# pasqal-io/Pulser

Measured on AMD Instinct MI355X. Metric: sim-us/sec, 14-atom Rydberg anneal sequence, sesolve fp64 (aggregate over independent sequences), higher is better.
Workload: dtype f64; 1 GPU; north star: 14-atom triangular register (2 x 7 at R_b), analog Ising anneal 3100 ns, sesolve complex128; step = the full 3.1 us for a batch of different sequences per GPU; n_atoms=14, sequences_per_gpu=256, parallelism=dp1

## Files before the change

pulser_amd/csrc/k_split_reg.hpp:

```cpp

#ifndef SPLITR_TRIG
#define SPLITR_TRIG 256
#endif
#ifndef SPLITR_KO
#define SPLITR_KO 0
#endif
#ifndef SPLITR_TMODE
#define SPLITR_TMODE 1
#endif
#ifndef SPLITR_GMODE
#define SPLITR_GMODE 0
#endif
#ifndef SPLITR_WMODE
#define SPLITR_WMODE 1
#endif
#ifndef SPLITR_EMODE
#define SPLITR_EMODE 0
#endif
#ifndef SPLITR_KWARM
#define SPLITR_KWARM 1
#endif
#ifndef SPLITR_PREF
#define SPLITR_PREF 0
#endif
#ifndef SPLITR_LATE
#define SPLITR_LATE 1
#endif
#ifndef SPLITR_P5
#define SPLITR_P5 0
#endif
#ifndef SPLITR_LATE_REAL
#define SPLITR_LATE_REAL 0
#endif
#ifndef SPLITR_YCHAIN
#define SPLITR_YCHAIN 1
#endif
#include "split_ychain.hpp"

template <int N, int NR>
struct SplitRegLayout {
  static constexpr int NW = N - 6 - NR;
  static constexpr int NTB = NR - NW;
  static constexpr int ND = 6 - NTB;
  static_assert(NW >= 0 && NW <= 3 && NTB >= 2 && ND >= 1 && ND <= 4, "unsupported shape");
  static constexpr bool kXchg = SPLITR_TMODE != 3;
  __host__ __device__ static constexpr int regbit(bool odd, int j) {
    if (!odd) return 6 + NW + j;
    return j < NW ? 6 + j : (kXchg ? ND + (j - NW) : 6 + NW + j);
  }
  __host__ __device__ static constexpr int lanebit(bool odd, int j) {
    if (j < ND || !odd || !kXchg) return j;
    return 6 + 2 * NW + (j - ND);
  }
  __host__ __device__ static constexpr int wavebit(bool odd, int j) { return odd ? 6 + NW + j : 6 + j; }
  __host__ __device__ static constexpr unsigned index(bool odd, unsigned t, unsigned r) {
    unsigned i = 0;
    for (int j = 0; j < 6; ++j) i |= ((t >> j) & 1u) << lanebit(odd, j);
    for (int j = 0; j < NW; ++j) i |= ((t >> (6 + j)) & 1u) << wavebit(odd, j);
    for (int j = 0; j < NR; ++j) i |= ((r >> j) & 1u) << regbit(odd, j);
    return i;
  }
  static constexpr int FM = ND == 4 ? 0 : (ND == 3 ? 2 : 3);
  __host__ __device__ static constexpr int swz(int y) { return ND == 3 ? ((y >> 1) & 1) : (y & FM); }
};

template <int I, int E, class Fn>
__device__ __forceinline__ void splitr_for(Fn&& f) {
  if constexpr (I < E) {
    f(std::integral_constant<int, I>{});
    splitr_for<I + 1, E>(f);
  }
}
template <int V>
using splitr_c = std::integral_constant<int, V>;
__host__ __device__ constexpr int splitr_low_clear(int v) {
  int j = 0;
  while (v & (1 << j)) ++j;
  return j;
}

template <int CTRL>
__device__ __forceinline__ double splitr_dpp(double v) {
  const int lo = __builtin_amdgcn_update_dpp(0, __double2loint(v), CTRL, 0xF, 0xF, true);
  const int hi = __builtin_amdgcn_update_dpp(0, __double2hiint(v), CTRL, 0xF, 0xF, true);
  return __hiloint2double(hi, lo);
}
#ifndef SPLITR_B2
#define SPLITR_B2 0
#endif
#ifndef SPLITR_HM
#define SPLITR_HM 1
#endif
template <int ND>
__device__ __forceinline__ unsigned splitr_lane(unsigned t) { return (SPLITR_HM && ND >= 3) ? t ^ ((t & 4u) ? 3u : 0u) : t; }
template <int F>
__device__ __forceinline__ double splitr_partner(double v) {
  if constexpr (F == 0) return splitr_dpp<0xB1>(v);
  else if constexpr (F == 1) return splitr_dpp<0x4E>(v);
  else if constexpr (F == 3) return splitr_dpp<0x128>(v);
  else if constexpr (SPLITR_HM == 1) return splitr_dpp<0x141>(v);
  else if constexpr (SPLITR_B2 == 1) {
    const int lo = __builtin_amdgcn_ds_swizzle(__double2loint(v), 0x101F);
    const int hi = __builtin_amdgcn_ds_swizzle(__double2hiint(v), 0x101F);
    return __hiloint2double(hi, lo);
  }
  else return splitr_dpp<0x1B>(splitr_dpp<0x141>(v));
}

template <int N, int NR, bool DECAY, bool ROWS = false, bool CPLX = false, bool SNAP = false>
__global__ __launch_bounds__(64 << (N - 6 - NR)) __attribute__((amdgpu_waves_per_eu(1, NR >= 6 ? 1 : 2))) void k_split_reg(const SplitArgs A, const SplitRun R, long long stage_stride) {
  static_assert(!(SNAP && (ROWS || DECAY)), "snapshots inside a run: plain ket runs only");
  typedef SplitRegLayout<N, NR> L;
  constexpr int NW = L::NW, NTB = L::NTB, ND = L::ND;
  constexpr int NT = 64 << NW;
  constexpr int NA = 1 << NR;
  constexpr int PW = (1 << NW) - 1;
  constexpr int CH = NA / 4;
  constexpr int NG = 1 << NW;
  constexpr int GR = 1 << NTB;
  constexpr int NBUF = CH / GR;
  extern __shared__ __attribute__((aligned(16))) char smem[];
  cplx* pbuf = reinterpret_cast<cplx*>(smem);
  cplx* trig = pbuf + 2 * NT * CH;
  cplx* gtab = trig + SPLITR_TRIG;
  double* wtab = reinterpret_cast<double*>(gtab + (NT / 64) * NA);
  double* etab = wtab + (SPLIT_MAX_SUB * SPLIT_MAX_STAGES + 2);

  const unsigned t = threadIdx.x;
  const unsigned l = t & 63u, w = t >> 6;
  const unsigned tq = splitr_lane<ND>(t);
  const int b = ROWS ? (int)blockIdx.z : (int)blockIdx.y;
  const int n_pre = R.kick_pre != 0.0 ? 1 : 0;
  const int n_stages = splitrun_first(R, R.nsub) + 1 + n_pre;
  const double csgn = (ROWS && A.conj) ? -1.0 : 1.0;
  const double* __restrict__ coefs = A.ccur + (size_t)b * N * 4;
  const double* __restrict__ e0 = A.e0 + (size_t)b * A.e0_stride;

  if (SPLITR_WMODE) {
    for (int jj = (int)t; jj < n_stages; jj += NT) {
      const int j = jj - n_pre;
      wtab[jj] = j < 0 ? 0.0 : splitrun_weight(R, j);
    }
  }
  for (unsigned k = t; k < SPLITR_TRIG; k += NT) {
    double sn, cs;
    sincospi((double)k * (2.0 / SPLITR_TRIG), &sn, &cs);
    trig[k] = make_double2(cs, sn);
  }
  double et[2], ev[2][NR], eg[2];
#pragma unroll
  for (int o = 0; o < 2; ++o) {
    et[o] = e0[L::index(o, tq, NA - 1)];
#pragma unroll
    for (int j = 0; j < NR; ++j) ev[o][j] = e0[L::index(o, tq, (NA - 1) ^ (1u << j))] - et[o];
    eg[o] = e0[L::index(o, NT - 1, l & (NA - 1))];
    if (SPLITR_EMODE) {
      etab[(2 * o) * NT + t] = et[o];
      etab[(2 * o + 1) * NT + t] = eg[o];
    }
  }
  double* ftl = etab + (SPLITR_EMODE ? 4 * NT : 0);
  unsigned a_row = 0;
  auto row_factor = [&](int which, unsigned col_bits, unsigned mask) -> double {
    const unsigned a = a_row;
    const int n11 = __popc(a & col_bits & mask), n10 = __popc(a & ~col_bits & mask), n01 = __popc(~a & col_bits & mask);
    const int n00 = __popc(mask) - n11 - n10 - n01;
    const double* tb = ftl + 64 * which;
    return tb[n00] * tb[16 + n01] * tb[32 + n10] * tb[48 + n11];
  };
  if (ROWS && (A.use_pre || A.use_post) && t < 128) ftl[t] = A.ftab[t];
  __syncthreads();
  typedef const __attribute__((address_space(4))) double* cptr_t;
  auto expmi = [&](double phi) -> cplx {
    const double kk = rint(phi * (SPLITR_TRIG / 6.283185307179586));
    double rr = fma(-kk, 6.283185307179586 / SPLITR_TRIG, phi);
    rr = fma(-kk, 2.4492935982947064e-16 / SPLITR_TRIG, rr);
    const cplx tb = trig[((int)kk) & (SPLITR_TRIG - 1)];
    const double r2 = rr * rr;
    double cr, sr;
    if (SPLITR_TRIG >= 512) {
      cr = fma(r2, fma(r2, 4.1666666666666664e-02, -0.5), 1.0);
      sr = rr * fma(r2, fma(r2, 8.333333333333333e-03, -1.6666666666666666e-01), 1.0);
    } else {
      cr = fma(r2, fma(r2, fma(r2, -1.3888888888888889e-03, 4.1666666666666664e-02), -0.5), 1.0);
      sr = rr * fma(r2, fma(r2, fma(r2, -1.984126984126984e-04, 8.333333333333333e-03), -1.6666666666666666e-01), 1.0);
    }
    return make_double2(fma(tb.x, cr, -tb.y * sr), -fma(tb.y, cr, tb.x * sr));
  };
  auto cm = [](cplx a, cplx c) -> cplx { return make_double2(fma(a.x, c.x, -a.y * c.y), fma(a.x, c.y, a.y * c.x)); };
  cplx* __restrict__ const tslice = pbuf + 64 * w;
  const unsigned la = l & ((1u << ND) - 1u), lT = l >> ND;

  for (unsigned row = ROWS ? blockIdx.y : 0u; row < (ROWS ? (1u << N) : 1u); row += ROWS ? gridDim.y : 1u) {
  a_row = row;
  cplx* __restrict__ st = A.state + ((((size_t)b << (ROWS ? N : 0)) + (ROWS ? row : 0u)) << N);
  if (ROWS) __syncthreads();
  if (ROWS && A.use_pre && t < NA) ftl[128 + t] = row_factor(0, L::index(false, 0u, t), L::index(false, 0u, NA - 1));
  if (ROWS && A.use_pre) __syncthreads();
  double xr[NA], xi[NA];
  {
    const double fl = (ROWS && A.use_pre) ? row_factor(0, L::index(false, tq, 0u), L::index(false, NT - 1, 0u)) : 1.0;
    splitr_for<0, NA>([&](auto Rc) {
      constexpr int r = decltype(Rc)::value;
      const cplx v = st[L::index(false, tq, r)];
      const double f = (ROWS && A.use_pre) ? fl * ftl[128 + r] : 1.0;
      xr[r] = v.x * f;
      xi[r] = v.y * (ROWS ? f * csgn : f);
    });
  }


  auto rot_reg = [&](auto J, double T, double U, auto MASK, auto VAL) {
    if (SPLITR_KO & 16) return;
    splitr_for<0, NA>([&](auto Rc) {
      constexpr int r = decltype(Rc)::value, j = decltype(J)::value;
      if constexpr ((r & decltype(MASK)::value) == decltype(VAL)::value && !(r & (1 << j))) {
        constexpr int q = r | (1 << j);
        const double a0x = xr[r], a0y = xi[r], a1x = xr[q], a1y = xi[q];
        if constexpr (CPLX) {
          xr[r] = fma(-U, a1x, fma(-T, a1y, a0x));
          xi[r] = fma(-U, a1y, fma(T, a1x, a0y));
          xr[q] = fma(U, a0x, fma(-T, a0y, a1x));
          xi[q] = fma(U, a0y, fma(T, a0x, a1y));
        } else {
          xr[r] = fma(-T, a1y, a0x);
          xi[r] = fma(T, a1x, a0y);
          xr[q] = fma(-T, a0y, a1x);
          xi[q] = fma(T, a0x, a1y);
        }
      }
    });
  };

  double cprod = 1.0;
  bool odd = false;
  double Dn[6 + NW + NR], wEn = 0.0;
  auto load_next = [&](int sn, bool oddn) {
    cptr_t cn = (cptr_t)(unsigned long long)(coefs + (size_t)sn * stage_stride);
#pragma unroll
    for (int j = 0; j < 6; ++j) Dn[j] = cn[4 * (N - 1 - (oddn ? L::lanebit(true, j) : L::lanebit(false, j))) + 3];
#pragma unroll
    for (int j = 0; j < NW; ++j) Dn[6 + j] = cn[4 * (N - 1 - (oddn ? L::wavebit(true, j) : L::wavebit(false, j))) + 3];
#pragma unroll
    for (int j = 0; j < NR; ++j) Dn[6 + NW + j] = cn[4 * (N - 1 - (oddn ? L::regbit(true, j) : L::regbit(false, j))) + 3];
    if (SPLITR_WMODE) wEn = uniform_d(wtab[sn]);
  };
  if (SPLITR_PREF) load_next(0, false);
  unsigned warm = 0;
  auto stage = [&](const int sg, auto plain_close_t) {
    constexpr bool PLAIN_CLOSE = decltype(plain_close_t)::value;
    cptr_t c4 = (cptr_t)(unsigned long long)(coefs + (size_t)sg * stage_stride);
    auto coef = [&](int bit_even, int bit_odd, int field) -> double {
      const int p = odd ? bit_odd : bit_even;
      return c4[4 * (N - 1 - p) + field];
    };
    double Tl[6], Dl[6], Tw[NW > 0 ? NW : 1], Dw[NW > 0 ? NW : 1], Tr[NR], Dr[NR];
    double Ul[6], Uw[NW > 0 ? NW : 1], Ur[NR];
    constexpr int TF = CPLX ? 2 : 1;
    double cnext = 1.0;
#pragma unroll
    for (int j = 0; j < 6; ++j) Dl[j] = SPLITR_PREF ? Dn[j] : coef(L::lanebit(false, j), L::lanebit(true, j), 3);
#pragma unroll
    for (int j = 0; j < NW; ++j) Dw[j] = SPLITR_PREF ? Dn[6 + j] : coef(L::wavebit(false, j), L::wavebit(true, j), 3);
#pragma unroll
    for (int j = 0; j < NR; ++j) Dr[j] = SPLITR_PREF ? Dn[6 + NW + j] : coef(L::regbit(false, j), L::regbit(true, j), 3);
    auto load_rot = [&](cptr_t cl) {
      auto coefl = [&](int bit_even, int bit_odd, int field) -> double {
        const int p = odd ? bit_odd : bit_even;
        return cl[4 * (N - 1 - p) + field];
      };
#pragma unroll
      for (int j = 0; j < 6; ++j) {
        Tl[j] = coefl(L::lanebit(false, j), L::lanebit(true, j), TF);
        Ul[j] = CPLX ? coefl(L::lanebit(false, j), L::lanebit(true, j), 1) : 0.0;
        cnext *= coefl(L::lanebit(false, j), L::lanebit(true, j), 0);
      }
#pragma unroll
      for (int j = 0; j < NW; ++j) {
        Tw[j] = coefl(L::wavebit(false, j), L::wavebit(true, j), TF);
        Uw[j] = CPLX ? coefl(L::wavebit(false, j), L::wavebit(true, j), 1) : 0.0;
        cnext *= coefl(L::wavebit(false, j), L::wavebit(true, j), 0);
      }
#pragma unroll
      for (int j = 0; j < NR; ++j) {
        Tr[j] = coefl(L::regbit(false, j), L::regbit(true, j), TF);
        Ur[j] = CPLX ? coefl(L::regbit(false, j), L::regbit(true, j), 1) : 0.0;
        cnext *= coefl(L::regbit(false, j), L::regbit(true, j), 0);
      }
    };
    constexpr bool kLate = (SPLITR_LATE && CPLX) || (SPLITR_LATE_REAL && !CPLX);
    if (!kLate && !PLAIN_CLOSE) load_rot(c4);
    double wE;
    if (SPLITR_WMODE && SPLITR_PREF) {
      wE = wEn;
    } else if (SPLITR_WMODE) {
      wE = uniform_d(wtab[sg]);
    } else {
      const int sj = sg - n_pre;
      wE = sj < 0 ? 0.0 : splitrun_weight(R, sj);
    }
    double et_s, eg_s;
    if (SPLITR_EMODE) {
      et_s = etab[(odd ? 2 : 0) * NT + t];
      eg_s = etab[(odd ? 3 : 1) * NT + t];
    } else {
      et_s = odd ? et[1] : et[0];
      eg_s = odd ? eg[1] : eg[0];
    }

    cplx Bf, F[NR], Gl;
    if (!(SPLITR_KO & 8)) {
      double dthr = 0.0;
#pragma unroll
      for (int j = 0; j < 6; ++j) dthr += ((tq >> j) & 1u) ? 0.0 : Dl[j];
#pragma unroll
      for (int j = 0; j < NW; ++j) dthr += ((tq >> (6 + j)) & 1u) ? 0.0 : Dw[j];
      Bf = expmi(fma(wE, et_s, -dthr));
      double sc = cprod;
      if (DECAY)
        sc *= exp(wE * (A.dec_a + A.dec_b * (double)(__popc(tq) + NR)));
      Bf = make_double2(Bf.x * sc, Bf.y * sc);
      const double dF = DECAY ? exp(-wE * A.dec_b) : 1.0;
#pragma unroll
      for (int j = 0; j < NR; ++j) {
        F[j] = expmi(fma(wE, odd ? ev[1][j] : ev[0][j], -Dr[j]));
        if (DECAY) F[j] = make_double2(F[j].x * dF, F[j].y * dF);
      }
      Gl = expmi(wE * eg_s);
      if (!SPLITR_GMODE) {
        gtab[w * NA + (l & (NA - 1))] = Gl;
        __builtin_amdgcn_wave_barrier();
      }
    }
    if (kLate && !PLAIN_CLOSE) {
      unsigned long long cl = (unsigned long long)(coefs + (size_t)sg * stage_stride);
      asm volatile("" : "+s"(cl));
      load_rot((cptr_t)cl);
    }
    cprod = cnext;
    const cplx* __restrict__ gw = gtab + w * NA;
    auto gval = [&](auto Rc) -> cplx {
      constexpr int r = decltype(Rc)::value;
      if (SPLITR_GMODE) {
        const int a = __builtin_amdgcn_readlane(__double2loint(Gl.x), r), b2 = __builtin_amdgcn_readlane(__double2hiint(Gl.x), r);
        const int c = __builtin_amdgcn_readlane(__double2loint(Gl.y), r), d = __builtin_amdgcn_readlane(__double2hiint(Gl.y), r);
        return make_double2(__hiloint2double(b2, a), __hiloint2double(d, c));
      }
      return gw[r];
    };

    cplx Pg[NG];
    auto phase_group = [&](auto Gc) {
      constexpr int g = decltype(Gc)::value;
      if (SPLITR_KO & 8) return;
      if constexpr (g == NG - 1) Pg[g] = Bf;
      else Pg[g] = cm(Pg[g | (1 << splitr_low_clear(g))], F[splitr_low_clear(g)]);
      cplx Pt[GR];
      splitr_for<0, GR>([&](auto Ic) {
        constexpr int rho = GR - 1 - decltype(Ic)::value;
        if constexpr (rho == GR - 1) Pt[rho] = Pg[g];
        else Pt[rho] = cm(Pt[rho | (1 << splitr_low_clear(rho))], F[NW + splitr_low_clear(rho)]);
        constexpr int r = g | (rho << NW);
        const cplx q = cm(Pt[rho], gval(splitr_c<r>{}));
        const double ax = xr[r], ay = xi[r];
        xr[r] = fma(ax, q.x, -ay * q.y);
        xi[r] = fma(ax, q.y, ay * q.x);
      });
    };
    constexpr bool kP5 = SPLITR_P5 && SPLITR_TMODE == 1 && NTB == 2 && NW > 0 && !(SPLITR_KO & 4);
    auto swap_d = [](double& a, double& c, auto is32) {
      unsigned alo = (unsigned)__double2loint(a), ahi = (unsigned)__double2hiint(a);
      unsigned clo = (unsigned)__double2loint(c), chi = (unsigned)__double2hiint(c);
      if constexpr (decltype(is32)::value) {
        auto p = __builtin_amdgcn_permlane32_swap(alo, clo, false, false);
        auto q = __builtin_amdgcn_permlane32_swap(ahi, chi, false, false);
        alo = p[0]; clo = p[1]; ahi = q[0]; chi = q[1];
      } else {
        auto p = __builtin_amdgcn_permlane16_swap(alo, clo, false, false);
        auto q = __builtin_amdgcn_permlane16_swap(ahi, chi, false, false);
        alo = p[0]; clo = p[1]; ahi = q[0]; chi = q[1];
      }
      a = __hiloint2double((int)ahi, (int)alo);
      c = __hiloint2double((int)chi, (int)clo);
    };
    constexpr bool kYChain = SPLITR_YCHAIN != 0 && !CPLX && SPLITR_HM == 1 && SPLITR_TMODE == 1 && !SPLITR_B2 && !(SPLITR_KO & 2) && ND >= 2;
    constexpr bool kYStore = kYChain && SPLITR_YCHAIN == 2 && NW > 0 && !kP5 && !(SPLITR_KO & 4);
    auto t_swap = [&](auto Gc) {
      constexpr int g = decltype(Gc)::value;
      if (SPLITR_KO & 1) return;
      constexpr int r0 = g, r1 = g | (1 << NW), r2 = g | (2 << NW), r3 = g | (3 << NW);
      swap_d(xr[r0], xr[r1], std::false_type{}); swap_d(xi[r0], xi[r1], std::false_type{});
      swap_d(xr[r2], xr[r3], std::false_type{}); swap_d(xi[r2], xi[r3], std::false_type{});
      if constexpr (!kP5) {
        swap_d(xr[r0], xr[r2], std::true_type{}); swap_d(xi[r0], xi[r2], std::true_type{});
        swap_d(xr[r1], xr[r3], std::true_type{}); swap_d(xi[r1], xi[r3], std::true_type{});
      }
    };
    auto t_write = [&](auto Gc) {
      constexpr int g = decltype(Gc)::value;
      if (SPLITR_KO & 1) return;
      splitr_for<0, GR>([&](auto Ic) {
        constexpr int rho = decltype(Ic)::value;
        constexpr int run = rho + (NBUF == 2 ? (g & 1) * GR : 0);
        tslice[64 * NG * run + la + ((lT ^ (unsigned)L::swz(rho)) << ND)] = make_double2(xr[g | (rho << NW)], xi[g | (rho << NW)]);
      });
    };
    auto t_read = [&](auto Gc) {
      constexpr int g = decltype(Gc)::value;
      if (SPLITR_KO & 1) return;
      __builtin_amdgcn_wave_barrier();
      const unsigned run = lT + (NBUF == 2 ? (g & 1) * GR : 0);
      splitr_for<0, GR>([&](auto Ic) {
        constexpr int rho = decltype(Ic)::value;
        const cplx v = tslice[64 * NG * run + la + (((unsigned)rho ^ (unsigned)L::swz((int)lT)) << ND)];
        xr[g | (rho << NW)] = v.x;
        xi[g | (rho << NW)] = v.y;
      });
    };
    auto rot_t_old = [&](auto Gc) {
      splitr_for<0, NTB>([&](auto Mc) {
        constexpr int m = decltype(Mc)::value;
        rot_reg(splitr_c<NW + m>{}, Tr[NW + m], Ur[NW + m], splitr_c<PW>{}, Gc);
      });
    };
    auto rot_t_new = [&](auto Gc) {
      splitr_for<0, (kP5 ? 1 : NTB)>([&](auto Mc) {
        constexpr int m = decltype(Mc)::value;
        rot_reg(splitr_c<NW + m>{}, Tl[ND + m], Ul[ND + m], splitr_c<PW>{}, Gc);
      });
    };
    double Us[6] = {0.0, 0.0, 0.0, 0.0, 0.0, 0.0};
    if constexpr (CPLX) {
#pragma unroll
      for (int j = 0; j < 6; ++j) Us[j] = ((tq >> j) & 1u) ? Ul[j] : -Ul[j];
    }
    auto xpartner = [&](double v, auto Jc) -> double {
      int lo = __double2loint(v), hi = __double2hiint(v);
      if constexpr (decltype(Jc)::value == 4) {
        lo = __builtin_amdgcn_ds_swizzle(lo, 0x401F);
        hi = __builtin_amdgcn_ds_swizzle(hi, 0x401F);
      } else {
        const int addr = (int)((l ^ 32u) << 2);
        lo = __builtin_amdgcn_ds_bpermute(addr, lo);
        hi = __builtin_amdgcn_ds_bpermute(addr, hi);
      }
      return __hiloint2double(hi, lo);
    };
    auto rot_lane_x = [&](auto Rc) {
      constexpr int r = decltype(Rc)::value;
      if (SPLITR_KO & 1) return;
      splitr_for<4, 6>([&](auto Jc) {
        constexpr int j = decltype(Jc)::value;
        const double T = Tl[j], px = xpartner(xr[r], Jc), py = xpartner(xi[r], Jc);
        if constexpr (CPLX) {
          xr[r] = fma(Us[j], px, fma(-T, py, xr[r]));
          xi[r] = fma(Us[j], py, fma(T, px, xi[r]));
        } else {
          xr[r] = fma(-T, py, xr[r]);
          xi[r] = fma(T, px, xi[r]);
        }
      });
    };
    auto rot_lane = [&](auto Rc, auto MASK) {
      constexpr int r = decltype(Rc)::value, mask = decltype(MASK)::value;
      if (SPLITR_KO & 2) return;
      if constexpr (ND > 0 && (mask & 1)) {
        const double T = Tl[0], px = splitr_partner<0>(xr[r]), py = splitr_partner<0>(xi[r]);
        if constexpr (CPLX) {
          xr[r] = fma(Us[0], px, fma(-T, py, xr[r]));
          xi[r] = fma(Us[0], py, fma(T, px, xi[r]));
        } else {
          xr[r] = fma(-T, py, xr[r]);
          xi[r] = fma(T, px, xi[r]);
        }
      }
      if constexpr (ND > 1 && (mask & 2)) {
        const double T = Tl[1], px = splitr_partner<1>(xr[r]), py = splitr_partner<1>(xi[r]);
        if constexpr (CPLX) {
          xr[r] = fma(Us[1], px, fma(-T, py, xr[r]));
          xi[r] = fma(Us[1], py, fma(T, px, xi[r]));
        } else {
          xr[r] = fma(-T, py, xr[r]);
          xi[r] = fma(T, px, xi[r]);
        }
      }
      if constexpr (ND > 3 && (mask & 8)) {
        const double T = Tl[3], px = splitr_partner<3>(xr[r]), py = splitr_partner<3>(xi[r]);
        if constexpr (CPLX) {
          xr[r] = fma(Us[3], px, fma(-T, py, xr[r]));
          xi[r] = fma(Us[3], py, fma(T, px, xi[r]));
        } else {
          xr[r] = fma(-T, py, xr[r]);
          xi[r] = fma(T, px, xi[r]);
        }
      }
      if constexpr (ND > 2 && (mask & 4)) {
        const double T = Tl[2], px = splitr_partner<2>(xr[r]), py = splitr_partner<2>(xi[r]);
        if constexpr (CPLX) {
          xr[r] = fma(Us[2], px, fma(-T, py, xr[r]));
          xi[r] = fma(Us[2], py, fma(T, px, xi[r]));
        } else {
          xr[r] = fma(-T, py, xr[r]);
          xi[r] = fma(T, px, xi[r]);
        }
      }
    };
    if constexpr (PLAIN_CLOSE) {
      splitr_for<0, NG>([&](auto Ic) { phase_group(splitr_c<(NG - 1 - decltype(Ic)::value)>{}); });
    } else {
    constexpr int TMASK = SPLITR_TMODE == 2 ? 3 : 0;
    constexpr int PMASK = ((1 << ND) - 1) & ~TMASK;
    if constexpr (SPLITR_TMODE == 2) {
      splitr_for<0, NG>([&](auto Ic) { phase_group(splitr_c<(NG - 1 - decltype(Ic)::value)>{}); });
      splitr_for<0, NG>([&](auto Ic) {
        constexpr int g = NG - 1 - decltype(Ic)::value;
        rot_t_old(splitr_c<g>{});
        splitr_for<0, GR>([&](auto Qc) { rot_lane(splitr_c<(g | (decltype(Qc)::value << NW))>{}, splitr_c<TMASK>{}); });
        t_write(splitr_c<g>{});
        t_read(splitr_c<g>{});
        if constexpr (g + 1 < NG) rot_t_new(splitr_c<g + 1>{});
      });
      rot_t_new(splitr_c<0>{});
    } else {
      splitr_for<0, NG>([&](auto Ic) {
        constexpr int g = NG - 1 - decltype(Ic)::value;
        phase_group(splitr_c<g>{});
        rot_t_old(splitr_c<g>{});
        if constexpr (SPLITR_TMODE == 3) {
        } else if constexpr (SPLITR_TMODE == 1 && NTB == 2) {
          t_swap(splitr_c<g>{});
          rot_t_new(splitr_c<g>{});
        } else {
          t_write(splitr_c<g>{});
          t_read(splitr_c<g>{});
          if constexpr (g + 1 < NG) rot_t_new(splitr_c<g + 1>{});
        }
      });
      if constexpr (!(SPLITR_TMODE == 1 && NTB == 2) && SPLITR_TMODE != 3) rot_t_new(splitr_c<0>{});
    }

    constexpr int CM = 3 << (NR - 2);
    auto pre_regs = [&](auto Cc) {
      constexpr int c = decltype(Cc)::value;
      splitr_for<0, NW>([&](auto Jc) { rot_reg(Jc, Tr[decltype(Jc)::value], Ur[decltype(Jc)::value], splitr_c<CM>{}, splitr_c<(c << (NR - 2))>{}); });
    };
    auto chain_step = [&](auto Cc, auto Ic) {
      constexpr int c = decltype(Cc)::value, i = decltype(Ic)::value;
      typedef SplitYPlan<ND, (kYStore ? 1 : 0)> PL;
      constexpr SplitYHop h = PL::hops[i];
      if constexpr (h.n > 0) splitr_for<0, CH>([&](auto Kc) { constexpr int r = decltype(Kc)::value | (c << (NR - 2)); xi[r] = splitr_dpp<h.ctrl[0]>(xi[r]); });
      if constexpr (h.n > 1) splitr_for<0, CH>([&](auto Kc) { constexpr int r = decltype(Kc)::value | (c << (NR - 2)); xi[r] = splitr_dpp<h.ctrl[1]>(xi[r]); });
      if constexpr (i < ND) {
        const double T = Tl[PL::order[i < ND ? i : 0]];
        splitr_for<0, CH>([&](auto Kc) {
          constexpr int r = decltype(Kc)::value | (c << (NR - 2));
          const double x0 = xr[r];
          xr[r] = fma(-T, xi[r], x0);
          xi[r] = fma(T, x0, xi[r]);
        });
      }
    };
    auto pre = [&](auto Cc) {
      constexpr int c = decltype(Cc)::value;
      pre_regs(Cc);
      if constexpr (kYChain) {
        splitr_for<0, ND + 1>([&](auto Ic) { chain_step(Cc, Ic); });
      } else {
        splitr_for<0, CH>([&](auto Kc) {
          rot_lane(splitr_c<(decltype(Kc)::value | (c << (NR - 2)))>{}, splitr_c<PMASK>{});
          if constexpr (SPLITR_TMODE == 3) rot_lane_x(splitr_c<(decltype(Kc)::value | (c << (NR - 2)))>{});
        });
      }
    };
    auto post = [&](auto Cc) {
      constexpr int c = decltype(Cc)::value;
      splitr_for<0, NW>([&](auto Jc) { rot_reg(Jc, Tw[decltype(Jc)::value], Uw[decltype(Jc)::value], splitr_c<CM>{}, splitr_c<(c << (NR - 2))>{}); });
    };
    auto pass_write_part = [&](auto Cc, auto K0c, auto K1c) {
      constexpr int c = decltype(Cc)::value, K0 = decltype(K0c)::value, K1 = decltype(K1c)::value;
      if constexpr (kYStore) {
        constexpr unsigned S = SplitYPlan<ND, 1>::final_shift;
        double* __restrict__ px = reinterpret_cast<double*>(pbuf + (c & 1) * (NT * CH) + t);
        double* __restrict__ py = reinterpret_cast<double*>(pbuf + (c & 1) * (NT * CH) + (t ^ S)) + 1;
        splitr_for<K0, K1>([&](auto Kc) {
          constexpr int k = decltype(Kc)::value, kp = k & PW, ks = k >> NW;
          px[2 * 64 * NG * (kp + NG * ks)] = xr[k | (c << (NR - 2))];
          py[2 * 64 * NG * (kp + NG * ks)] = xi[k | (c << (NR - 2))];
        });
        return;
      }
      cplx* __restrict__ pb = pbuf + (c & 1) * (NT * CH) + t;
      splitr_for<K0, K1>([&](auto Kc) {
        constexpr int k = decltype(Kc)::value, kp = k & PW, ks = k >> NW;
        pb[64 * NG * (kp + NG * ks)] = make_double2(xr[k | (c << (NR - 2))], xi[k | (c << (NR - 2))]);
      });
    };
    auto pass_write = [&](auto Cc) { pass_write_part(Cc, splitr_c<0>{}, splitr_c<CH>{}); };
    auto write_pre = [&](auto Cw, auto Cp) {
      if constexpr (kYChain) {
        pre_regs(Cp);
        splitr_for<0, ND + 1>([&](auto Ic) {
          constexpr int i = decltype(Ic)::value;
          pass_write_part(Cw, splitr_c<(i * CH / (ND + 1))>{}, splitr_c<((i + 1) * CH / (ND + 1))>{});
          __builtin_amdgcn_sched_barrier(0);
          chain_step(Cp, Ic);
          __builtin_amdgcn_sched_barrier(0);
        });
      } else {
        pass_write(Cw);
        pre(Cp);
      }
    };
    auto pass_read = [&](auto Cc) {
      constexpr int c = decltype(Cc)::value;
      const cplx* __restrict__ pb = pbuf + (c & 1) * (NT * CH) + l + 64 * NG * w;
      splitr_for<0, CH>([&](auto Kc) {
        constexpr int k = decltype(Kc)::value, kp = k & PW, ks = k >> NW;
        const cplx v = pb[64 * (kp + NG * NG * ks)];
        xr[k | (c << (NR - 2))] = v.x;
        xi[k | (c << (NR - 2))] = v.y;
      });
    };
    typedef splitr_c<0> C0; typedef splitr_c<1> C1; typedef splitr_c<2> C2; typedef splitr_c<3> C3;
    auto pass_write5 = [&](auto Sc) {
      constexpr int S = decltype(Sc)::value;
      cplx* __restrict__ pb = pbuf + t;
      splitr_for<0, 2 * CH>([&](auto Kc) {
        constexpr int k = decltype(Kc)::value, kp = k & PW, t1 = k >> NW;
        constexpr int r = kp | (S << (NR - 2)) | (t1 << (NR - 1));
        pb[64 * NG * (kp + NG * t1)] = make_double2(xr[r], xi[r]);
      });
    };
    auto pass_read5 = [&](auto Sc) {
      constexpr int S = decltype(Sc)::value;
      const cplx* __restrict__ pb = pbuf + (l & 31u) + 64 * NG * (w + NG * (l >> 5));
      splitr_for<0, 2 * CH>([&](auto Kc) {
        constexpr int k = decltype(Kc)::value, kp = k & PW, t1 = k >> NW;
        constexpr int r = kp | (S << (NR - 2)) | (t1 << (NR - 1));
        const cplx v = pb[32 * t1 + 64 * kp];
        xr[r] = v.x;
        xi[r] = v.y;
      });
    };
    auto pre5 = [&](auto Sc) {
      constexpr int S = decltype(Sc)::value;
      pre(splitr_c<S>{}); pre(splitr_c<S + 2>{});
    };
    auto post5 = [&](auto Sc) {
      constexpr int S = decltype(Sc)::value;
      post(splitr_c<S>{}); post(splitr_c<S + 2>{});
      rot_reg(splitr_c<NW + 1>{}, Tl[ND + 1], Ul[ND + 1], splitr_c<(1 << (NR - 2))>{}, splitr_c<(S << (NR - 2))>{});
    };
    if constexpr (kP5) {
      static_assert(CH == (1 << NW), "SPLITR_P5: chunks of 2^NW registers");
      pre5(C0{});
      __syncthreads();
      pass_write5(C0{});
      pre5(C1{});
      __syncthreads();
      pass_read5(C0{});
      if (SPLITR_KWARM) {
        typedef const __attribute__((address_space(4))) unsigned* uptr_t;
        uptr_t nx = (uptr_t)(unsigned long long)(coefs + (size_t)(sg + 1 < n_stages ? sg + 1 : sg) * stage_stride);
#pragma unroll
        for (int k = 0; k < 8; ++k) warm ^= nx[k < 7 ? 16 * k : 8 * N - 1];
      }
      __syncthreads();
      pass_write5(C1{});
      post5(C0{});
      __syncthreads();
      pass_read5(C1{});
      if (SPLITR_PREF) load_next(sg + 1 < n_stages ? sg + 1 : sg, !odd);
      post5(C1{});
    } else if constexpr (NW == 0 || (SPLITR_KO & 4)) {
      pre(C0{}); pre(C1{}); pre(C2{}); pre(C3{});
      post(C0{}); post(C1{}); post(C2{}); post(C3{});
    } else {
      pre(C0{});
      write_pre(C0{}, C1{});
      __syncthreads();
      pass_read(C0{});
      if (SPLITR_KWARM) {
        typedef const __attribute__((address_space(4))) unsigned* uptr_t;
        uptr_t nx = (uptr_t)(unsigned long long)(coefs + (size_t)(sg + 1 < n_stages ? sg + 1 : sg) * stage_stride);
#pragma unroll
        for (int k = 0; k < 8; ++k) warm ^= nx[k < 7 ? 16 * k : 8 * N - 1];
      }
      write_pre(C1{}, C2{});
      __syncthreads();
      pass_read(C1{});
      write_pre(C2{}, C3{});
      __syncthreads();
      pass_read(C2{});
      pass_write(C3{});
      post(C0{});
      post(C1{});
      __syncthreads();
      pass_read(C3{});
      if (SPLITR_PREF) load_next(sg + 1 < n_stages ? sg + 1 : sg, !odd);
      post(C2{});
      post(C3{});
    }
    odd = !odd;
    }
    if (SPLITR_KWARM) asm volatile("" ::"s"(warm));
  };
  const int n_full = R.kick_post == 0.0 ? n_stages - 1 : n_stages;
  if constexpr (SNAP) {
    int snap_at = splitrun_first(R, 1) + n_pre - 1, snap_sub = 0;
    for (int sg = 0; sg < n_full; ++sg) {
      stage(sg, std::false_type{});
      if (sg == snap_at) {
        const int slot = R.snap[snap_sub];
        const long long moff = (slot >= 0 && A.snap_map_slots > 0) ? A.snap_map[(size_t)b * A.snap_map_slots + slot] : 0;
        if (slot >= 0 && moff >= 0) {
          unsigned lw = odd ? L::index(true, tq, 0u) : L::index(false, tq, 0u);
          asm volatile("" : "+v"(lw));
          cplx* __restrict__ sd = A.snap_map_slots > 0 ? A.snaps + ((size_t)moff << N)
                                             : A.snaps + (size_t)slot * A.snap_stride + ((size_t)b << N);
          if (odd) {
            splitr_for<0, NA>([&](auto Rc) {
              constexpr int r = decltype(Rc)::value;
              __builtin_nontemporal_store(xr[r], &sd[lw + L::index(true, 0u, r)].x);
              __builtin_nontemporal_store(xi[r], &sd[lw + L::index(true, 0u, r)].y);
            });
          } else {
            splitr_for<0, NA>([&](auto Rc) {
              constexpr int r = decltype(Rc)::value;
              __builtin_nontemporal_store(xr[r], &sd[lw + L::index(false, 0u, r)].x);
              __builtin_nontemporal_store(xi[r], &sd[lw + L::index(false, 0u, r)].y);
            });
          }
        }
        ++snap_sub;
        snap_at = snap_sub < R.nsub ? splitrun_first(R, snap_sub + 1) + n_pre - 1 : (1 << 30);
      }
    }
  } else {
    for (int sg = 0; sg < n_full; ++sg) stage(sg, std::false_type{});
  }
  if (n_full < n_stages) stage(n_stages - 1, std::true_type{});
  double fl = (ROWS && n_full == n_stages) ? cprod : 1.0;
  if (ROWS && n_full == n_stages && !A.use_post) {
    splitr_for<0, NA>([&](auto Rc) {
      constexpr int r = decltype(Rc)::value;
      xr[r] *= fl;
      xi[r] *= fl;
    });
  }
  if (ROWS && A.use_post) {
    __syncthreads();
    if (t < NA) ftl[128 + t] = row_factor(1, odd ? L::index(true, 0u, t) : L::index(false, 0u, t), odd ? L::index(true, 0u, NA - 1) : L::index(false, 0u, NA - 1));
    __syncthreads();
    fl *= row_factor(1, odd ? L::index(true, tq, 0u) : L::index(false, tq, 0u), odd ? L::index(true, NT - 1, 0u) : L::index(false, NT - 1, 0u));
  }
  bool stored = false;
  if constexpr (!ROWS) {
    if (A.dst || A.dst2 || A.cmp) {
      stored = true;
      const size_t boff = (size_t)b << N;
      cplx* __restrict__ out = A.dst ? A.dst + boff : st;
      cplx* __restrict__ out2 = A.dst2 ? A.dst2 + boff : nullptr;
      const cplx* __restrict__ ref = A.cmp ? A.cmp + boff : nullptr;
      const unsigned lw = odd ? L::index(true, tq, 0u) : L::index(false, tq, 0u);
      double dmax = 0.0, dsum = 0.0;
      auto put = [&](unsigned ix, double vx, double vy) {
        const cplx v = make_double2(vx, vy);
        out[ix] = v;
        if (out2) out2[ix] = v;
        if (ref) {
          const cplx c = ref[ix];
          const double dx = vx - c.x, dy = vy - c.y;
          const double d2 = fma(dx, dx, dy * dy);
          dmax = fmax(dmax, d2);
          dsum += d2;
        }
      };
      if (odd) {
        splitr_for<0, NA>([&](auto Rc) { constexpr int r = decltype(Rc)::value; put(lw + L::index(true, 0u, r), xr[r], xi[r]); });
      } else {
        splitr_for<0, NA>([&](auto Rc) { constexpr int r = decltype(Rc)::value; put(lw + L::index(false, 0u, r), xr[r], xi[r]); });
      }
      if (ref) {
        for (int o = 32; o > 0; o >>= 1) {
          dmax = fmax(dmax, __shfl_xor(dmax, o, 64));
          dsum += __shfl_xor(dsum, o, 64);
        }
        double* red = reinterpret_cast<double*>(gtab);
        __syncthreads();
        if (l == 0) { red[2 * w] = dmax; red[2 * w + 1] = dsum; }
        __syncthreads();
        if (t == 0) {
          double m = red[0], sm = red[1];
          for (int k = 1; k < NT / 64; ++k) { m = fmax(m, red[2 * k]); sm += red[2 * k + 1]; }
          A.cmp_err[b] = m;
          A.cmp_err[gridDim.y + b] = sm;
        }
      }
    }
  }
  if (!stored) {
  splitr_for<0, NA>([&](auto Rc) {
    constexpr int r = decltype(Rc)::value;
    const double f = (ROWS && A.use_post) ? fl * ftl[128 + r] : 1.0;
    st[odd ? L::index(true, tq, r) : L::index(false, tq, r)] = make_double2(xr[r] * f, xi[r] * (ROWS ? f * csgn : f));
  });
  }
  }
}
```

Measured before the change: 12550 sim-us/s.

## Split expmi into table fetch and finish, prefetch G values and coefficient warm-up earlier

After: 13370 sim-us/s, median of 6. 1.07x the previous value.

```diff
diff --git a/pulser_amd/csrc/k_split_reg.hpp b/pulser_amd/csrc/k_split_reg.hpp
--- a/pulser_amd/csrc/k_split_reg.hpp
+++ b/pulser_amd/csrc/k_split_reg.hpp
@@ -18,7 +18,10 @@
 #define SPLITR_EMODE 0
 #endif
 #ifndef SPLITR_KWARM
-#define SPLITR_KWARM 1
+#define SPLITR_KWARM 2
+#endif
+#ifndef SPLITR_GAHEAD
+#define SPLITR_GAHEAD 1
 #endif
 #ifndef SPLITR_PREF
 #define SPLITR_PREF 0
@@ -171,11 +174,13 @@
   if (ROWS && (A.use_pre || A.use_post) && t < 128) ftl[t] = A.ftab[t];
   __syncthreads();
   typedef const __attribute__((address_space(4))) double* cptr_t;
-  auto expmi = [&](double phi) -> cplx {
+  auto expmi_arg = [&](double phi, double& rr) -> cplx {
     const double kk = rint(phi * (SPLITR_TRIG / 6.283185307179586));
-    double rr = fma(-kk, 6.283185307179586 / SPLITR_TRIG, phi);
+    rr = fma(-kk, 6.283185307179586 / SPLITR_TRIG, phi);
     rr = fma(-kk, 2.4492935982947064e-16 / SPLITR_TRIG, rr);
-    const cplx tb = trig[((int)kk) & (SPLITR_TRIG - 1)];
+    return trig[((int)kk) & (SPLITR_TRIG - 1)];
+  };
+  auto expmi_fin = [&](double rr, cplx tb) -> cplx {
     const double r2 = rr * rr;
     double cr, sr;
     if (SPLITR_TRIG >= 512) {
@@ -186,6 +191,11 @@
       sr = rr * fma(r2, fma(r2, fma(r2, -1.984126984126984e-04, 8.333333333333333e-03), -1.6666666666666666e-01), 1.0);
     }
     return make_double2(fma(tb.x, cr, -tb.y * sr), -fma(tb.y, cr, tb.x * sr));
+  };
+  auto expmi = [&](double phi) -> cplx {
+    double rr;
+    const cplx tb = expmi_arg(phi, rr);
+    return expmi_fin(rr, tb);
   };
   auto cm = [](cplx a, cplx c) -> cplx { return make_double2(fma(a.x, c.x, -a.y * c.y), fma(a.x, c.y, a.y * c.x)); };
   cplx* __restrict__ const tslice = pbuf + 64 * w;
@@ -247,6 +257,8 @@
   };
   if (SPLITR_PREF) load_next(0, false);
   unsigned warm = 0;
+  unsigned warm_v = 0, warm_va = 0;
+  const unsigned long long stage_bytes = (unsigned long long)stage_stride * sizeof(double);
   auto stage = [&](const int sg, auto plain_close_t) {
     constexpr bool PLAIN_CLOSE = decltype(plain_close_t)::value;
     cptr_t c4 = (cptr_t)(unsigned long long)(coefs + (size_t)sg * stage_stride);
@@ -309,18 +321,49 @@
     }
 
     cplx Bf, F[NR], Gl;
+    constexpr bool kGAhead = SPLITR_GAHEAD != 0 && !SPLITR_GMODE && SPLITR_TMODE == 1 && NTB == 2 && !CPLX && !ROWS && !PLAIN_CLOSE && !(SPLITR_KO & 8);
+    cplx Gq[GR];
+    auto g_fetch = [&](auto Gc) {
+      constexpr int g = decltype(Gc)::value;
+      const cplx* __restrict__ gq = gtab + w * NA;
+      splitr_for<0, GR>([&](auto Ic) {
+        constexpr int rho = GR - 1 - decltype(Ic)::value;
+        Gq[rho] = gq[g | (rho << NW)];
+      });
+    };
     if (!(SPLITR_KO & 8)) {
       double dthr = 0.0;
 #pragma unroll
       for (int j = 0; j < 6; ++j) dthr += ((tq >> j) & 1u) ? 0.0 : Dl[j];
 #pragma unroll
       for (int j = 0; j < NW; ++j) dthr += ((tq >> (6 + j)) & 1u) ? 0.0 : Dw[j];
-      Bf = expmi(fma(wE, et_s, -dthr));
       double sc = cprod;
       if (DECAY)
         sc *= exp(wE * (A.dec_a + A.dec_b * (double)(__popc(tq) + NR)));
+      const double dF = DECAY ? exp(-wE * A.dec_b) : 1.0;
+      if constexpr (kGAhead) {
+        double rB, rF[NR], rG;
+        const cplx tG = expmi_arg(wE * eg_s, rG);
+        const cplx tB = expmi_arg(fma(wE, et_s, -dthr), rB);
+        cplx tF[NR];
+#pragma unroll
+        for (int j = 0; j < NR; ++j) tF[j] = expmi_arg(fma(wE, odd ? ev[1][j] : ev[0][j], -Dr[j]), rF[j]);
+        __builtin_amdgcn_sched_barrier(0);
+        Gl = expmi_fin(rG, tG);
+        gtab[w * NA + (l & (NA - 1))] = Gl;
+        __builtin_amdgcn_wave_barrier();
+        g_fetch(splitr_c<NG - 1>{});
+        __builtin_amdgcn_sched_barrier(0);
+        Bf = expmi_fin(rB, tB);
+        Bf = make_double2(Bf.x * sc, Bf.y * sc);
+#pragma unroll
+        for (int j = 0; j < NR; ++j) {
+          F[j] = expmi_fin(rF[j], tF[j]);
+          if (DECAY) F[j] = make_double2(F[j].x * dF, F[j].y * dF);
+        }
+      } else {
+      Bf = expmi(fma(wE, et_s, -dthr));
       Bf = make_double2(Bf.x * sc, Bf.y * sc);
-      const double dF = DECAY ? exp(-wE * A.dec_b) : 1.0;
 #pragma unroll
       for (int j = 0; j < NR; ++j) {
         F[j] = expmi(fma(wE, odd ? ev[1][j] : ev[0][j], -Dr[j]));
@@ -330,6 +373,7 @@
       if (!SPLITR_GMODE) {
         gtab[w * NA + (l & (NA - 1))] = Gl;
         __builtin_amdgcn_wave_barrier();
+      }
       }
     }
     if (kLate && !PLAIN_CLOSE) {
@@ -353,6 +397,14 @@
     auto phase_group = [&](auto Gc) {
       constexpr int g = decltype(Gc)::value;
       if (SPLITR_KO & 8) return;
+      cplx Gg[GR];
+      if constexpr (kGAhead) {
+        splitr_for<0, GR>([&](auto Ic) { Gg[decltype(Ic)::value] = Gq[decltype(Ic)::value]; });
+        if constexpr (SPLITR_GAHEAD == 1 && g > 0) {
+          g_fetch(splitr_c<(g > 0 ? g - 1 : 0)>{});
+          __builtin_amdgcn_sched_barrier(0);
+        }
+      }
       if constexpr (g == NG - 1) Pg[g] = Bf;
       else Pg[g] = cm(Pg[g | (1 << splitr_low_clear(g))], F[splitr_low_clear(g)]);
       cplx Pt[GR];
@@ -361,11 +413,18 @@
         if constexpr (rho == GR - 1) Pt[rho] = Pg[g];
         else Pt[rho] = cm(Pt[rho | (1 << splitr_low_clear(rho))], F[NW + splitr_low_clear(rho)]);
         constexpr int r = g | (rho << NW);
-        const cplx q = cm(Pt[rho], gval(splitr_c<r>{}));
+        cplx gv;
+        if constexpr (kGAhead) gv = Gg[rho];
+        else gv = gval(splitr_c<r>{});
+        const cplx q = cm(Pt[rho], gv);
         const double ax = xr[r], ay = xi[r];
         xr[r] = fma(ax, q.x, -ay * q.y);
         xi[r] = fma(ax, q.y, ay * q.x);
       });
+      if constexpr (kGAhead && SPLITR_GAHEAD == 2 && g > 0) {
+        g_fetch(splitr_c<(g > 0 ? g - 1 : 0)>{});
+        __builtin_amdgcn_sched_barrier(0);
+      }
     };
     constexpr bool kP5 = SPLITR_P5 && SPLITR_TMODE == 1 && NTB == 2 && NW > 0 && !(SPLITR_KO & 4);
     auto swap_d = [](double& a, double& c, auto is32) {
@@ -508,6 +567,28 @@
     if constexpr (PLAIN_CLOSE) {
       splitr_for<0, NG>([&](auto Ic) { phase_group(splitr_c<(NG - 1 - decltype(Ic)::value)>{}); });
     } else {
+    unsigned wv[8];
+    constexpr bool kWarmLate = (SPLITR_KWARM == 2 || SPLITR_KWARM == 3) && !kP5 && NW > 0 && !(SPLITR_KO & 4);
+    constexpr bool kWarmInLoop = kWarmLate && SPLITR_TMODE == 1 && NTB == 2 && !CPLX;
+    auto warm_issue = [&]() {
+      const unsigned long long nv = (unsigned long long)c4 + (sg + 1 < n_stages ? stage_bytes : 0ull);
+      unsigned long long na = ((unsigned long long)(unsigned)__builtin_amdgcn_readfirstlane((int)(nv >> 32)) << 32) |
+                              (unsigned)__builtin_amdgcn_readfirstlane((int)nv);
+      __builtin_amdgcn_sched_barrier(0);
+      asm volatile("" : "+s"(na));
+      if constexpr (SPLITR_KWARM == 2) {
+        typedef const __attribute__((address_space(4))) unsigned* uptr_t;
+        uptr_t nx = (uptr_t)na;
+#pragma unroll
+        for (int k = 0; k < 8; ++k) wv[k] = nx[k < 7 ? 16 * k : 8 * N - 1];
+      } else {
+        warm_va ^= warm_v;
+        const unsigned k = l & 7u;
+        typedef const __attribute__((address_space(1))) unsigned* gptr_t;
+        warm_v = ((gptr_t)na)[k < 7u ? 16u * k : 8u * N - 1u];
+      }
+      __builtin_amdgcn_sched_barrier(0);
+    };
     constexpr int TMASK = SPLITR_TMODE == 2 ? 3 : 0;
     constexpr int PMASK = ((1 << ND) - 1) & ~TMASK;
     if constexpr (SPLITR_TMODE == 2) {
@@ -525,6 +606,7 @@
       splitr_for<0, NG>([&](auto Ic) {
         constexpr int g = NG - 1 - decltype(Ic)::value;
         phase_group(splitr_c<g>{});
+        if constexpr (g == 0 && kWarmInLoop) warm_issue();
         rot_t_old(splitr_c<g>{});
         if constexpr (SPLITR_TMODE == 3) {
         } else if constexpr (SPLITR_TMODE == 1 && NTB == 2) {
@@ -676,11 +758,19 @@
       pre(C0{}); pre(C1{}); pre(C2{}); pre(C3{});
       post(C0{}); post(C1{}); post(C2{}); post(C3{});
     } else {
+      if constexpr (kWarmLate && !kWarmInLoop) warm_issue();
       pre(C0{});
       write_pre(C0{}, C1{});
+      if constexpr (SPLITR_KWARM == 2) {
+#pragma unroll
+        for (int k = 0; k < 8; ++k) {
+          asm volatile("" : "+s"(wv[k]));
+          warm ^= wv[k];
+        }
+      }
       __syncthreads();
       pass_read(C0{});
-      if (SPLITR_KWARM) {
+      if (SPLITR_KWARM == 1) {
         typedef const __attribute__((address_space(4))) unsigned* uptr_t;
         uptr_t nx = (uptr_t)(unsigned long long)(coefs + (size_t)(sg + 1 < n_stages ? sg + 1 : sg) * stage_stride);
 #pragma unroll
@@ -704,6 +794,7 @@
     odd = !odd;
     }
     if (SPLITR_KWARM) asm volatile("" ::"s"(warm));
+    if constexpr (SPLITR_KWARM == 3) asm volatile("" ::"v"(warm_va));
   };
   const int n_full = R.kick_post == 0.0 ? n_stages - 1 : n_stages;
   if constexpr (SNAP) {
@@ -739,6 +830,7 @@
   } else {
     for (int sg = 0; sg < n_full; ++sg) stage(sg, std::false_type{});
   }
+  if (SPLITR_KWARM == 3) asm volatile("" ::"v"(warm_v));
   if (n_full < n_stages) stage(n_stages - 1, std::true_type{});
   double fl = (ROWS && n_full == n_stages) ? cprod : 1.0;
   if (ROWS && n_full == n_stages && !A.use_post) {
```
